# VisionDepth/VisionDepth3D

Measured on NVIDIA H100. Metric: end-to-end frames/sec (depth+stereo), higher is better.
Workload: dtype f16 GEMM operands, fp32 accumulate; DIBR fp32

## Files before the change

visiondepth3d_b200/csrc/depth_kernels.cu:

```cuda
#include <stdlib.h>

#include "depth_launch.h"
#include "umma_gemm.cuh"
#include "umma_attention.cuh"

namespace vd3d {

__global__ void __launch_bounds__(256) k_layernorm(const float* __restrict__ x, int rows, int D,
                                                   const float* __restrict__ gamma, const float* __restrict__ beta,
                                                   __half* __restrict__ out, int row_off, float eps) {
  int row = blockIdx.x * 8 + (threadIdx.x >> 5);
  int lane = threadIdx.x & 31;
  if (row >= rows) return;
  const float4* xr = (const float4*)(x + (size_t)(row + row_off) * D);
  float4 v[8];
  const int n = D / 128;
  float s = 0.f;
#pragma unroll
  for (int i = 0; i < 8; ++i)
    if (i < n) {
      v[i] = xr[lane + 32 * i];
      s += (v[i].x + v[i].y) + (v[i].z + v[i].w);
    }
  for (int o = 16; o; o >>= 1) s += __shfl_xor_sync(0xffffffffu, s, o);
  const float mean = s / (float)D;
  float q = 0.f;
#pragma unroll
  for (int i = 0; i < 8; ++i)
    if (i < n) {
      float a = v[i].x - mean, b = v[i].y - mean, c = v[i].z - mean, d = v[i].w - mean;
      q += (a * a + b * b) + (c * c + d * d);
    }
  for (int o = 16; o; o >>= 1) q += __shfl_xor_sync(0xffffffffu, q, o);
  const float rstd = rsqrtf(q / (float)D + eps);
  uint2* orow = (uint2*)(out + (size_t)row * D);
#pragma unroll
  for (int i = 0; i < 8; ++i)
    if (i < n) {
      const int c4 = lane + 32 * i;
      float4 g4 = ((const float4*)gamma)[c4], b4 = ((const float4*)beta)[c4];
      __half2 h0 = __floats2half2_rn((v[i].x - mean) * rstd * g4.x + b4.x, (v[i].y - mean) * rstd * g4.y + b4.y);
      __half2 h1 = __floats2half2_rn((v[i].z - mean) * rstd * g4.z + b4.z, (v[i].w - mean) * rstd * g4.w + b4.w);
      uint2 u;
      u.x = *(uint32_t*)&h0;
      u.y = *(uint32_t*)&h1;
      orow[c4] = u;
    }
}

__global__ void __launch_bounds__(256) k_patch_im2col(const float* __restrict__ px, int IH, int IW, int ph, int pw,
                                                      __half* __restrict__ A, int kpad) {
  int idx = blockIdx.x * 256 + threadIdx.x;
  int total = ph * pw * 588;
  if (idx >= total) return;
  int k = idx % 588, t = idx / 588;
  int c = k / 196, rr = k % 196, dy = rr / 14, dx = rr % 14;
  int py = t / pw, pxx = t % pw;
  float v = px[((size_t)c * IH + (py * 14 + dy)) * IW + (pxx * 14 + dx)];
  A[(size_t)t * kpad + k] = __float2half_rn(v);
}

__global__ void k_set_cls(float* __restrict__ x, const float* __restrict__ cls, const float* __restrict__ pos, int D) {
  int i = blockIdx.x * 256 + threadIdx.x;
  if (i < D) x[i] = cls[i] + pos[i];
}

__global__ void __launch_bounds__(256) k_im2col_s2(const __half* __restrict__ in, int H, int W, int C, int ldc,
                                                   __half* __restrict__ out, int OH, int OW) {
  size_t idx = (size_t)blockIdx.x * 256 + threadIdx.x;
  size_t total = (size_t)OH * OW * 9 * C;
  if (idx >= total) return;
  int c = idx % C;
  size_t r = idx / C;
  int tap = r % 9;
  size_t o = r / 9;
  int ox = o % OW, oy = o / OW;
  int iy = oy * 2 - 1 + tap / 3, ix = ox * 2 - 1 + tap % 3;
  __half v = __float2half_rn(0.f);
  if (iy >= 0 && iy < H && ix >= 0 && ix < W) v = in[((size_t)iy * W + ix) * ldc + c];
  out[idx] = v;
}

__global__ void __launch_bounds__(256) k_upsample_ac(const __half* __restrict__ in, int H, int W, int C,
                                                     __half* __restrict__ out, int OH, int OW) {
  size_t idx = (size_t)blockIdx.x * 256 + threadIdx.x;
  int c8 = C / 8;
  size_t total = (size_t)OH * OW * c8;
  if (idx >= total) return;
  int cg = idx % c8;
  size_t o = idx / c8;
  int ox = o % OW, oy = o / OW;
  float sy = (OH > 1) ? (float)(H - 1) / (float)(OH - 1) : 0.f;
  float sx = (OW > 1) ? (float)(W - 1) / (float)(OW - 1) : 0.f;
  float fy = sy * oy, fx = sx * ox;
  int y0 = (int)fy, x0 = (int)fx;
  int y1 = min(y0 + 1, H - 1), x1 = min(x0 + 1, W - 1);
  float ly = fy - y0, lx = fx - x0;
  const uint4* p00 = (const uint4*)(in + ((size_t)y0 * W + x0) * C) + cg;
  const uint4* p01 = (const uint4*)(in + ((size_t)y0 * W + x1) * C) + cg;
  const uint4* p10 = (const uint4*)(in + ((size_t)y1 * W + x0) * C) + cg;
  const uint4* p11 = (const uint4*)(in + ((size_t)y1 * W + x1) * C) + cg;
  uint4 a = *p00, b = *p01, c = *p10, d = *p11, r;
  const __half2* ha = (const __half2*)&a;
  const __half2* hb = (const __half2*)&b;
  const __half2* hc = (const __half2*)&c;
  const __half2* hd = (const __half2*)&d;
  __half2* hr = (__half2*)&r;
#pragma unroll
  for (int j = 0; j < 4; ++j) {
    float2 fa = __half22float2(ha[j]), fb = __half22float2(hb[j]), fc = __half22float2(hc[j]),
           fd = __half22float2(hd[j]);
    float t0x = fa.x + lx * (fb.x - fa.x), t0y = fa.y + lx * (fb.y - fa.y);
    float t1x = fc.x + lx * (fd.x - fc.x), t1y = fc.y + lx * (fd.y - fc.y);
    hr[j] = __floats2half2_rn(t0x + ly * (t1x - t0x), t0y + ly * (t1y - t0y));
  }
  ((uint4*)(out + o * C))[cg] = r;
}

__global__ void __launch_bounds__(256) k_relu_f16(const __half* __restrict__ in, __half* __restrict__ out, size_t n8) {
  size_t i = (size_t)blockIdx.x * 256 + threadIdx.x;
  if (i >= n8) return;
  uint4 a = ((const uint4*)in)[i];
  __half2* h = (__half2*)&a;
  const __half2 z = __floats2half2_rn(0.f, 0.f);
#pragma unroll
  for (int j = 0; j < 4; ++j) h[j] = __hmax2(h[j], z);
  ((uint4*)out)[i] = a;
}

__device__ __forceinline__ float cubic_aa(float x) {
  const float a = -0.5f;
  x = fabsf(x);
  if (x < 1.0f) return ((a + 2.0f) * x - (a + 3.0f)) * x * x + 1.0f;
  if (x < 2.0f) return (((x - 5.0f) * x + 8.0f) * x - 4.0f) * a;
  return 0.0f;
}

__global__ void __launch_bounds__(256) k_resize_aa_u8(const uint8_t* __restrict__ src, int IH, int IW,
                                                      uint8_t* __restrict__ dst, int OH, int OW, int axis_y,
                                                      int bgr_to_rgb) {
  int ox = blockIdx.x * 32 + (threadIdx.x & 31);
  int oy = blockIdx.y * 8 + (threadIdx.x >> 5);
  if (ox >= OW || oy >= OH) return;
  const int in_sz = axis_y ? IH : IW, out_sz = axis_y ? OH : OW, o = axis_y ? oy : ox;
  float scale = (float)in_sz / (float)out_sz;
  float support = (scale >= 1.0f) ? 2.0f * scale : 2.0f;
  float invscale = (scale >= 1.0f) ? 1.0f / scale : 1.0f;
  float center = scale * ((float)o + 0.5f);
  int xmin = max(0, (int)(center - support + 0.5f));
  int xmax = min(in_sz, (int)(center + support + 0.5f));
  float wsum = 0.f, acc[3] = {0.f, 0.f, 0.f};
  for (int j = xmin; j < xmax; ++j) {
    float w = cubic_aa(((float)j - center + 0.5f) * invscale);
    wsum += w;
    const uint8_t* q = axis_y ? src + ((size_t)j * IW + ox) * 3 : src + ((size_t)oy * IW + j) * 3;
    acc[0] += w * (float)q[0];
    acc[1] += w * (float)q[1];
    acc[2] += w * (float)q[2];
  }
  uint8_t* d = dst + ((size_t)oy * OW + ox) * 3;
#pragma unroll
  for (int c = 0; c < 3; ++c) {
    float v = acc[c] / wsum;
    int iv = __float2int_rn(v);
    iv = iv < 0 ? 0 : (iv > 255 ? 255 : iv);
    d[bgr_to_rgb ? 2 - c : c] = (uint8_t)iv;
  }
}

__global__ void __launch_bounds__(256) k_normalize_px(const uint8_t* __restrict__ rgb, int H, int W,
                                                      float* __restrict__ px) {
  int i = blockIdx.x * 256 + threadIdx.x;
  if (i >= H * W) return;
  const float mean[3] = {0.485f, 0.456f, 0.406f}, stdv[3] = {0.229f, 0.224f, 0.225f};
#pragma unroll
  for (int c = 0; c < 3; ++c) {
    float v = (float)rgb[(size_t)i * 3 + c] * (1.0f / 255.0f);
    px[(size_t)c * H * W + i] = (v - mean[c]) / stdv[c];
  }
}

__device__ __forceinline__ void cubic_coeffs(float t, float* c) {
  const float A = -0.75f;
  float x;
  x = t + 1.0f;
  c[0] = ((A * x - 5.0f * A) * x + 8.0f * A) * x - 4.0f * A;
  x = t;
  c[1] = ((A + 2.0f) * x - (A + 3.0f)) * x * x + 1.0f;
  x = 1.0f - t;
  c[2] = ((A + 2.0f) * x - (A + 3.0f)) * x * x + 1.0f;
  x = 2.0f - t;
  c[3] = ((A * x - 5.0f * A) * x + 8.0f * A) * x - 4.0f * A;
}
__device__ __forceinline__ unsigned f2ord(float f) {
  unsigned u = __float_as_uint(f);
  return (u & 0x80000000u) ? ~u : (u | 0x80000000u);
}
__device__ __forceinline__ float ord2f(unsigned u) {
  return __uint_as_float((u & 0x80000000u) ? (u & 0x7FFFFFFFu) : ~u);
}
__global__ void __launch_bounds__(256) k_depth_upsample_minmax(const float* __restrict__ d, int IH, int IW,
                                                               float* __restrict__ out, int OH, int OW,
                                                               unsigned* __restrict__ mm) {
  int ox = blockIdx.x * 32 + (threadIdx.x & 31);
  int oy = blockIdx.y * 8 + (threadIdx.x >> 5);
  float v = 0.f;
  bool ok = ox < OW && oy < OH;
  if (ok) {
    if (IH == OH && IW == OW) {
      v = d[(size_t)oy * IW + ox];
    } else {
      float sy = (float)IH / (float)OH, sx = (float)IW / (float)OW;
      float fy = sy * ((float)oy + 0.5f) - 0.5f, fx = sx * ((float)ox + 0.5f) - 0.5f;
      int iy = (int)floorf(fy), ix = (int)floorf(fx);
      float cy[4], cx[4];
      cubic_coeffs(fy - (float)iy, cy);
      cubic_coeffs(fx - (float)ix, cx);
      v = 0.f;
#pragma unroll
      for (int j = 0; j < 4; ++j) {
        int yy = min(max(iy - 1 + j, 0), IH - 1);
        float r = 0.f;
#pragma unroll
        for (int i = 0; i < 4; ++i) {
          int xx = min(max(ix - 1 + i, 0), IW - 1);
          r += cx[i] * d[(size_t)yy * IW + xx];
        }
        v += cy[j] * r;
      }
    }
    out[(size_t)oy * OW + ox] = v;
  }
  __shared__ float slo[8], shi[8];
  float lo = ok ? v : INFINITY, hi = ok ? v : -INFINITY;
  for (int o = 16; o; o >>= 1) {
    lo = fminf(lo, __shfl_xor_sync(0xffffffffu, lo, o));
    hi = fmaxf(hi, __shfl_xor_sync(0xffffffffu, hi, o));
  }
  if ((threadIdx.x & 31) == 0) {
    slo[threadIdx.x >> 5] = lo;
    shi[threadIdx.x >> 5] = hi;
  }
  __syncthreads();
  if (threadIdx.x == 0) {
    for (int i = 1; i < 8; ++i) {
      lo = fminf(lo, slo[i]);
      hi = fmaxf(hi, shi[i]);
    }
    if (lo <= hi) {
      atomicMin(&mm[0], f2ord(lo));
      atomicMax(&mm[1], f2ord(hi));
    }
  }
}
__global__ void k_minmax_reset(unsigned* mm) {
  mm[0] = 0xFFFFFFFFu;
  mm[1] = 0u;
}
__global__ void __launch_bounds__(256) k_depth_to_u8(const float* __restrict__ d, int n, const unsigned* __restrict__ mm,
                                                     uint8_t* __restrict__ out, int invert) {
  int i = blockIdx.x * 256 + threadIdx.x;
  if (i >= n) return;
  float lo = ord2f(mm[0]), hi = ord2f(mm[1]);
  float v = ((d[i] - lo) / (hi - lo + 1e-6f)) * 255.0f;
  int iv = (int)v;
  iv = iv < 0 ? 0 : (iv > 255 ? 255 : iv);
  out[i] = (uint8_t)(invert ? 255 - iv : iv);
}

__global__ void __launch_bounds__(256) k_add_relu_f16(const __half* __restrict__ a, const __half* __restrict__ b,
                                                      __half* __restrict__ sum, __half* __restrict__ sum_relu,
                                                      size_t n8) {
  size_t i = (size_t)blockIdx.x * 256 + threadIdx.x;
  if (i >= n8) return;
  uint4 ua = ((const uint4*)a)[i], ub = ((const uint4*)b)[i], us, ur;
  const __half2* ha = (const __half2*)&ua;
  const __half2* hb = (const __half2*)&ub;
  __half2* hs = (__half2*)&us;
  __half2* hr = (__half2*)&ur;
#pragma unroll
  for (int j = 0; j < 4; ++j) {
    float2 fa = __half22float2(ha[j]), fb = __half22float2(hb[j]);
    float sx = fa.x + fb.x, sy = fa.y + fb.y;
    hs[j] = __floats2half2_rn(sx, sy);
    hr[j] = __floats2half2_rn(fmaxf(sx, 0.f), fmaxf(sy, 0.f));
  }
  ((uint4*)sum)[i] = us;
  ((uint4*)sum_relu)[i] = ur;
}

void launch_preprocess(const uint8_t* frame_bgr, int H, int W, uint8_t* tmp_u8, uint8_t* rgb_u8, float* px, int OH,
                       int OW, cudaStream_t s) {
  dim3 g1((OW + 31) / 32, (H + 7) / 8), g2((OW + 31) / 32, (OH + 7) / 8);
  k_resize_aa_u8<<<g1, 256, 0, s>>>(frame_bgr, H, W, tmp_u8, H, OW, 0, 0);
  k_resize_aa_u8<<<g2, 256, 0, s>>>(tmp_u8, H, OW, rgb_u8, OH, OW, 1, 1);
  k_normalize_px<<<(OH * OW + 255) / 256, 256, 0, s>>>(rgb_u8, OH, OW, px);
}
void launch_depth_post(const float* depth, int IH, int IW, float* up, int OH, int OW, unsigned* mm, uint8_t* out_u8,
                       int invert, cudaStream_t s) {
  k_minmax_reset<<<1, 1, 0, s>>>(mm);
  dim3 g((OW + 31) / 32, (OH + 7) / 8);
  k_depth_upsample_minmax<<<g, 256, 0, s>>>(depth, IH, IW, up, OH, OW, mm);
  if (out_u8) k_depth_to_u8<<<(OH * OW + 255) / 256, 256, 0, s>>>(up, OH * OW, mm, out_u8, invert);
}
void launch_add_relu_f16(const __half* a, const __half* b, __half* sum, __half* sum_relu, size_t n, cudaStream_t s) {
  size_t n8 = n / 8;
  k_add_relu_f16<<<(unsigned)((n8 + 255) / 256), 256, 0, s>>>(a, b, sum, sum_relu, n8);
}
void launch_layernorm(const float* x, int rows, int D, const float* g, const float* b, __half* out, int row_off,
                      cudaStream_t s) {
  k_layernorm<<<(rows + 7) / 8, 256, 0, s>>>(x, rows, D, g, b, out, row_off, 1e-6f);
}
void launch_patch_im2col(const float* px, int IH, int IW, int ph, int pw, __half* A, int kpad, cudaStream_t s) {
  int total = ph * pw * 588;
  k_patch_im2col<<<(total + 255) / 256, 256, 0, s>>>(px, IH, IW, ph, pw, A, kpad);
}
void launch_set_cls(float* x, const float* cls, const float* pos, int D, cudaStream_t s) {
  k_set_cls<<<(D + 255) / 256, 256, 0, s>>>(x, cls, pos, D);
}
void launch_im2col_s2(const __half* in, int H, int W, int C, int ldc, __half* out, int OH, int OW, cudaStream_t s) {
  size_t total = (size_t)OH * OW * 9 * C;
  k_im2col_s2<<<(unsigned)((total + 255) / 256), 256, 0, s>>>(in, H, W, C, ldc, out, OH, OW);
}
void launch_upsample_ac(const __half* in, int H, int W, int C, __half* out, int OH, int OW, cudaStream_t s) {
  size_t total = (size_t)OH * OW * (C / 8);
  k_upsample_ac<<<(unsigned)((total + 255) / 256), 256, 0, s>>>(in, H, W, C, out, OH, OW);
}
__global__ void __launch_bounds__(256) k_sr_in(const uint8_t* __restrict__ bgr, __half* __restrict__ x, int npix) {
  int i = blockIdx.x * 256 + threadIdx.x;
  if (i >= npix) return;
  const uint8_t* q = bgr + (size_t)i * 3;
  uint4 z = make_uint4(0, 0, 0, 0);
  uint4* dst = (uint4*)(x + (size_t)i * 64);
  __align__(16) __half h4[8];
  h4[0] = __float2half_rn((float)q[2] / 255.0f);
  h4[1] = __float2half_rn((float)q[1] / 255.0f);
  h4[2] = __float2half_rn((float)q[0] / 255.0f);
#pragma unroll
  for (int k = 3; k < 8; ++k) h4[k] = __float2half_rn(0.f);
  dst[0] = *(uint4*)h4;
#pragma unroll
  for (int k = 1; k < 8; ++k) dst[k] = z;
}
__global__ void __launch_bounds__(256) k_sr_out(const float* __restrict__ conv, int ldc, const uint8_t* __restrict__ bgr,
                                                uint8_t* __restrict__ out, int h, int w) {
  int X = blockIdx.x * 32 + (threadIdx.x & 31);
  int Y = blockIdx.y * 8 + (threadIdx.x >> 5);
  if (X >= 4 * w || Y >= 4 * h) return;
  const int y = Y >> 2, x = X >> 2, sub = (Y & 3) * 4 + (X & 3);
  const float* cv = conv + ((size_t)y * w + x) * ldc + sub;
  const uint8_t* q = bgr + ((size_t)y * w + x) * 3;
  uint8_t* o = out + ((size_t)Y * 4 * w + X) * 3;
#pragma unroll
  for (int c = 0; c < 3; ++c) {
    float v = cv[c * 16] + ((float)q[2 - c] / 255.0f);
    v = fminf(fmaxf(v, 0.f), 1.f) * 255.0f;
    o[2 - c] = (uint8_t)(int)v;
  }
}
void launch_sr_in(const uint8_t* bgr, __half* x, int npix, cudaStream_t s) {
  k_sr_in<<<(npix + 255) / 256, 256, 0, s>>>(bgr, x, npix);
}
void launch_sr_out(const float* conv, int ldc, const uint8_t* bgr, uint8_t* out, int h, int w, cudaStream_t s) {
  dim3 g((4 * w + 31) / 32, (4 * h + 7) / 8);
  k_sr_out<<<g, 256, 0, s>>>(conv, ldc, bgr, out, h, w);
}

void launch_relu_f16(const __half* in, __half* out, size_t n, cudaStream_t s) {
  size_t n8 = n / 8;
  k_relu_f16<<<(unsigned)((n8 + 255) / 256), 256, 0, s>>>(in, out, n8);
}

template <int BN, int STAGES>
static cudaError_t launch_gemm_t(const CUtensorMap& a, const CUtensorMap& b, const GemmArgs& g, dim3 grid,
                                 cudaStream_t s) {
  static bool attr_set = false;
  constexpr int smem = GemmSmem<BN, STAGES>::kTotal;
  if (!attr_set) {
    cudaError_t e = cudaFuncSetAttribute(k_umma_gemm<BN, STAGES>, cudaFuncAttributeMaxDynamicSharedMemorySize, smem);
    if (e != cudaSuccess) return e;
    attr_set = true;
  }
  k_umma_gemm<BN, STAGES><<<grid, kGemmThreads, smem, s>>>(a, b, g);
  return cudaGetLastError();
}

cudaError_t launch_attention(const CUtensorMap& q, const CUtensorMap& k, const CUtensorMap& v, int ntok, int dmodel,
                             __half* out, int heads, int images, int npad, cudaStream_t s) {
  static bool attr_set = false;
  if (!attr_set) {
    cudaError_t e = cudaFuncSetAttribute(k_umma_attention, cudaFuncAttributeMaxDynamicSharedMemorySize, kAttnSmem);
    if (e != cudaSuccess) return e;
    attr_set = true;
  }
  AttnArgs a;
  a.ntok = ntok;
  a.dmodel = dmodel;
  a.out = out;
  a.heads = heads;
  a.npad = npad;
  dim3 grid((ntok + 127) / 128, heads * images);
  k_umma_attention<<<grid, kAttnThreads, kAttnSmem, s>>>(q, k, v, a);
  return cudaGetLastError();
}

static int sm_count() {
  static int sms = 0;
  if (!sms) {
    int dev = 0;
    cudaGetDevice(&dev);
    if (cudaDeviceGetAttribute(&sms, cudaDevAttrMultiProcessorCount, dev) != cudaSuccess || sms <= 0) sms = 132;
  }
  return sms;
}

cudaError_t launch_gemm_variant(int variant, const CUtensorMap& a, const CUtensorMap& b, const GemmArgs& g_in,
                                int m_tiles, int batch, cudaStream_t s) {
  GemmArgs g = g_in;
  g.nt = (g.N + 127) / 128;
  g.mt = m_tiles;
  g.nz = batch;
  const int total = g.nt * g.mt * g.nz, sms = sm_count();
  dim3 grid(total < sms ? total : sms, 1, 1);
  switch (variant) {
    case 0: return launch_gemm_t<128, 4>(a, b, g, grid, s);
    case 1: return launch_gemm_t<128, 3>(a, b, g, grid, s);
    case 2: return launch_gemm_t<128, 2>(a, b, g, grid, s);
    default: return cudaErrorInvalidValue;
  }
}

cudaError_t launch_gemm(int bn, const CUtensorMap& a, const CUtensorMap& b, const GemmArgs& g_in, int m_tiles,
                        int batch, cudaStream_t s) {
  GemmArgs g = g_in;
  g.nt = (g.N + bn - 1) / bn;
  g.mt = m_tiles;
  g.nz = batch;
  const int total = g.nt * g.mt * g.nz, sms = sm_count();
  dim3 grid(total < sms ? total : sms, 1, 1);
  switch (bn) {
    case 128: return launch_gemm_t<128, 4>(a, b, g, grid, s);
    case 64: return launch_gemm_t<64, 6>(a, b, g, grid, s);
    case 32: return launch_gemm_t<32, 6>(a, b, g, grid, s);
    default: return cudaErrorInvalidValue;
  }
}

}
```

visiondepth3d_b200/csrc/umma_attention.cuh:

```cuda
#pragma once
#include "umma_gemm.cuh"

namespace vd3d {

struct AttnArgs {
  int ntok;
  int dmodel;
  __half* out;
  int heads;
  int npad;
};

constexpr int kAttnThreads = 384;
constexpr int kAttnKS = 2;
constexpr int kAttnSmem = 16384  + kAttnKS * (16384  + 16384 ) + 1024  + 256 ;

namespace umma {
__device__ __forceinline__ float quad_max(float x) {
  x = fmaxf(x, __shfl_xor_sync(0xffffffffu, x, 1));
  return fmaxf(x, __shfl_xor_sync(0xffffffffu, x, 2));
}
__device__ __forceinline__ float quad_sum(float x) {
  x += __shfl_xor_sync(0xffffffffu, x, 1);
  return x + __shfl_xor_sync(0xffffffffu, x, 2);
}
__device__ __forceinline__ uint32_t pack_h2(float a, float b) {
  __half2 h = __floats2half2_rn(a, b);
  return *(uint32_t*)&h;
}
}

__global__ void __launch_bounds__(kAttnThreads, 1)
k_umma_attention(const __grid_constant__ CUtensorMap tmQ, const __grid_constant__ CUtensorMap tmK,
                 const __grid_constant__ CUtensorMap tmV, const AttnArgs g) {
  extern __shared__ uint8_t smem_raw[];
  const uint32_t sm = (umma::smem_u32(smem_raw) + 1023u) & ~1023u;
  const uint32_t sQ = sm, sK = sm + 16384, sV = sK + kAttnKS * 16384;
  const uint32_t bars = sV + kAttnKS * 16384;
  const uint32_t q_full = bars, kv_full = bars + 8, kv_empty = kv_full + 8 * kAttnKS;

  const int warp = threadIdx.x >> 5, lane = threadIdx.x & 31;
  const int qblk = blockIdx.x, zq = blockIdx.y, h = zq % g.heads, img = zq / g.heads;
  const int T = (g.ntok + 127) / 128;

  if (warp == 0 && lane == 0) {
    umma::prefetch_tmap(&tmQ);
    umma::prefetch_tmap(&tmK);
    umma::prefetch_tmap(&tmV);
    umma::mbar_init(q_full, 1);
    for (int i = 0; i < kAttnKS; ++i) {
      umma::mbar_init(kv_full + 8 * i, 1);
      umma::mbar_init(kv_empty + 8 * i, 2);
    }
    umma::fence_barrier_init();
  }
  __syncthreads();

  if (warp < 4) {
    if (warp == 0 && lane == 0) {
      umma::mbar_expect_tx(q_full, 16384);
      umma::tma_load_3d(sQ, &tmQ, q_full, 0, qblk * 128, zq);
      for (int t = 0; t < T; ++t) {
        const int ks = t % kAttnKS;
        umma::mbar_wait(kv_empty + 8 * ks, ((t / kAttnKS) & 1) ^ 1);
        const uint32_t fb = kv_full + 8 * ks;
        umma::mbar_expect_tx(fb, 32768);
        umma::tma_load_3d(sK + ks * 16384, &tmK, fb, 0, t * 128, zq);
        const uint32_t dst = sV + ks * 16384;
        umma::tma_load_3d(dst, &tmV, fb, t * 128, 0, zq);
        umma::tma_load_3d(dst + 8192, &tmV, fb, t * 128 + 64, 0, zq);
      }
    }
    return;
  }

  const int wg = (warp >> 2) - 1;
  const int wq = warp & 3;
  const float L2E = 1.4426950408889634f;
  const int cq = 2 * (lane & 3);
  float o[32];
#pragma unroll
  for (int i = 0; i < 32; ++i) o[i] = 0.f;
  float m_run[2] = {-INFINITY, -INFINITY}, l_run[2] = {0.f, 0.f};

  umma::mbar_wait(q_full, 0);
  const uint64_t dq = umma::make_desc(sQ + (uint32_t)(wg * 64 * 128));
  for (int t = 0; t < T; ++t) {
    const int ks = t % kAttnKS;
    umma::mbar_wait(kv_full + 8 * ks, (t / kAttnKS) & 1);
    float s[64];
    {
      const uint64_t dk = umma::make_desc(sK + ks * 16384);
      umma::wgmma_fence();
#pragma unroll
      for (int k = 0; k < 4; ++k) umma::wgmma_m64n128_ss(s, dq + (uint64_t)(2 * k), dk + (uint64_t)(2 * k), k ? 1u : 0u);
      umma::wgmma_commit();
      umma::wgmma_wait<0>();
      umma::fence_regs(s);
    }
    const int nvalid = g.ntok - t * 128;
    float mx[2] = {-INFINITY, -INFINITY};
#pragma unroll
    for (int j = 0; j < 16; ++j)
#pragma unroll
      for (int i = 0; i < 4; ++i) {
        if (nvalid < 128 && 8 * j + cq + (i & 1) >= nvalid) s[4 * j + i] = -INFINITY;
        mx[i >> 1] = fmaxf(mx[i >> 1], s[4 * j + i]);
      }
    float scale[2], mref[2];
#pragma unroll
    for (int rr = 0; rr < 2; ++rr) {
      const float m_new = fmaxf(m_run[rr], umma::quad_max(mx[rr]) * L2E);
      scale[rr] = umma::ex2_fast(m_run[rr] - m_new);
      m_run[rr] = m_new;
      mref[rr] = m_new - 8.0f;
    }
    float ls[2] = {0.f, 0.f};
    uint32_t p[32];
#pragma unroll
    for (int j = 0; j < 16; ++j) {
      const float p0 = umma::ex2_fast(fmaf(s[4 * j + 0], L2E, -mref[0]));
      const float p1 = umma::ex2_fast(fmaf(s[4 * j + 1], L2E, -mref[0]));
      const float p2 = umma::ex2_fast(fmaf(s[4 * j + 2], L2E, -mref[1]));
      const float p3 = umma::ex2_fast(fmaf(s[4 * j + 3], L2E, -mref[1]));
      p[2 * j] = umma::pack_h2(p0, p1);
      p[2 * j + 1] = umma::pack_h2(p2, p3);
      const float2 h0 = __half22float2(*(const __half2*)&p[2 * j]), h1 = __half22float2(*(const __half2*)&p[2 * j + 1]);
      ls[0] += h0.x + h0.y;
      ls[1] += h1.x + h1.y;
    }
#pragma unroll
    for (int rr = 0; rr < 2; ++rr) l_run[rr] = l_run[rr] * scale[rr] + ls[rr];
#pragma unroll
    for (int j = 0; j < 8; ++j) {
      o[4 * j + 0] *= scale[0];
      o[4 * j + 1] *= scale[0];
      o[4 * j + 2] *= scale[1];
      o[4 * j + 3] *= scale[1];
    }
    umma::fence_regs(o);
    umma::wgmma_fence();
#pragma unroll
    for (int kk = 0; kk < 8; ++kk) {
      const uint32_t a[4] = {p[4 * kk], p[4 * kk + 1], p[4 * kk + 2], p[4 * kk + 3]};
      const uint64_t db = umma::make_desc(sV + ks * 16384 + (kk >> 2) * 8192) + (uint64_t)(2 * (kk & 3));
      umma::wgmma_m64n64_rs(o, a, db, 1u);
    }
    umma::wgmma_commit();
    umma::wgmma_wait<0>();
    umma::fence_regs(o);
    if ((threadIdx.x & 127) == 0) umma::mbar_arrive(kv_empty + 8 * ks);
  }

  float inv[2];
#pragma unroll
  for (int rr = 0; rr < 2; ++rr) inv[rr] = 1.0f / umma::quad_sum(l_run[rr]);
  const int r0 = qblk * 128 + wg * 64 + wq * 16 + (lane >> 2);
#pragma unroll
  for (int rr = 0; rr < 2; ++rr) {
    const int m = r0 + 8 * rr;
    if (m >= g.ntok) continue;
    __half* dst = g.out + ((size_t)img * g.npad + m) * g.dmodel + h * 64 + cq;
#pragma unroll
    for (int j = 0; j < 8; ++j)
      *(uint32_t*)(dst + 8 * j) = umma::pack_h2(o[4 * j + 2 * rr] * inv[rr], o[4 * j + 2 * rr + 1] * inv[rr]);
  }
}

}
```

Baseline: 318.6.

## Make attention persistent with QK/PV software pipelining and register rebalancing

```diff
diff --git a/visiondepth3d_b200/csrc/depth_kernels.cu b/visiondepth3d_b200/csrc/depth_kernels.cu
--- a/visiondepth3d_b200/csrc/depth_kernels.cu
+++ b/visiondepth3d_b200/csrc/depth_kernels.cu
@@ -385,6 +385,16 @@
   return cudaGetLastError();
 }
 
+static int sm_count() {
+  static int sms = 0;
+  if (!sms) {
+    int dev = 0;
+    cudaGetDevice(&dev);
+    if (cudaDeviceGetAttribute(&sms, cudaDevAttrMultiProcessorCount, dev) != cudaSuccess || sms <= 0) sms = 132;
+  }
+  return sms;
+}
+
 cudaError_t launch_attention(const CUtensorMap& q, const CUtensorMap& k, const CUtensorMap& v, int ntok, int dmodel,
                              __half* out, int heads, int images, int npad, cudaStream_t s) {
   static bool attr_set = false;
@@ -399,19 +409,9 @@
   a.out = out;
   a.heads = heads;
   a.npad = npad;
-  dim3 grid((ntok + 127) / 128, heads * images);
-  k_umma_attention<<<grid, kAttnThreads, kAttnSmem, s>>>(q, k, v, a);
+  a.items = (ntok + 127) / 128 * heads * images;
+  k_umma_attention<<<std::min(a.items, sm_count()), kAttnThreads, kAttnSmem, s>>>(q, k, v, a);
   return cudaGetLastError();
-}
-
-static int sm_count() {
-  static int sms = 0;
-  if (!sms) {
-    int dev = 0;
-    cudaGetDevice(&dev);
-    if (cudaDeviceGetAttribute(&sms, cudaDevAttrMultiProcessorCount, dev) != cudaSuccess || sms <= 0) sms = 132;
-  }
-  return sms;
 }
 
 cudaError_t launch_gemm_variant(int variant, const CUtensorMap& a, const CUtensorMap& b, const GemmArgs& g_in,
diff --git a/visiondepth3d_b200/csrc/umma_attention.cuh b/visiondepth3d_b200/csrc/umma_attention.cuh
--- a/visiondepth3d_b200/csrc/umma_attention.cuh
+++ b/visiondepth3d_b200/csrc/umma_attention.cuh
@@ -9,11 +9,16 @@
   __half* out;
   int heads;
   int npad;
+  int items;
 };
 
 constexpr int kAttnThreads = 384;
-constexpr int kAttnKS = 2;
-constexpr int kAttnSmem = 16384  + kAttnKS * (16384  + 16384 ) + 1024  + 256 ;
+constexpr int kAttnKS = 3;
+constexpr int kAttnSmem = 2 * 16384  + kAttnKS * (16384  + 16384 ) + 1024  +
+                          256 ;
+constexpr int kAttnProducerRegs = 24;
+constexpr int kAttnConsumerRegs = 240;
+static_assert(128 * kAttnProducerRegs + 256 * kAttnConsumerRegs <= 384 * 168, "register file overcommitted");
 
 namespace umma {
 __device__ __forceinline__ float quad_max(float x) {
@@ -27,6 +32,73 @@
 __device__ __forceinline__ uint32_t pack_h2(float a, float b) {
   __half2 h = __floats2half2_rn(a, b);
   return *(uint32_t*)&h;
+}
+
+__device__ __forceinline__ void attn_qk(float (&s)[64], uint64_t dq, uint32_t sk) {
+  const uint64_t dk = make_desc(sk);
+#pragma unroll
+  for (int k = 0; k < 4; ++k) wgmma_m64n128_ss(s, dq + (uint64_t)(2 * k), dk + (uint64_t)(2 * k), k ? 1u : 0u);
+}
+__device__ __forceinline__ void attn_pv(float (&o)[32], const uint32_t (&p)[32], uint32_t sv) {
+#pragma unroll
+  for (int kk = 0; kk < 8; ++kk) {
+    const uint32_t a[4] = {p[4 * kk], p[4 * kk + 1], p[4 * kk + 2], p[4 * kk + 3]};
+    const uint64_t db = make_desc(sv + (kk >> 2) * 8192) + (uint64_t)(2 * (kk & 3));
+    wgmma_m64n64_rs(o, a, db, 1u);
+  }
+}
+template <bool kMask>
+__device__ __forceinline__ void attn_softmax(float (&s)[64], int nvalid, int cq, float (&m_run)[2], float (&l_run)[2],
+                                             float (&scale)[2]) {
+  const float L2E = 1.4426950408889634f;
+  float mx[2] = {-INFINITY, -INFINITY};
+#pragma unroll
+  for (int j = 0; j < 16; ++j)
+#pragma unroll
+    for (int i = 0; i < 4; ++i) {
+      if (kMask && 8 * j + cq + (i & 1) >= nvalid) s[4 * j + i] = -INFINITY;
+      mx[i >> 1] = fmaxf(mx[i >> 1], s[4 * j + i]);
+    }
+  float mref[2];
+#pragma unroll
+  for (int rr = 0; rr < 2; ++rr) {
+    const float m_new = fmaxf(m_run[rr], quad_max(mx[rr]) * L2E);
+    scale[rr] = ex2_fast(m_run[rr] - m_new);
+    m_run[rr] = m_new;
+    mref[rr] = m_new - 8.0f;
+  }
+  float ls[2] = {0.f, 0.f};
+#pragma unroll
+  for (int j = 0; j < 16; ++j) {
+    const float p0 = ex2_fast(fmaf(s[4 * j + 0], L2E, -mref[0]));
+    const float p1 = ex2_fast(fmaf(s[4 * j + 1], L2E, -mref[0]));
+    const float p2 = ex2_fast(fmaf(s[4 * j + 2], L2E, -mref[1]));
+    const float p3 = ex2_fast(fmaf(s[4 * j + 3], L2E, -mref[1]));
+    const uint32_t u0 = pack_h2(p0, p1), u1 = pack_h2(p2, p3);
+    const float2 h0 = __half22float2(*(const __half2*)&u0), h1 = __half22float2(*(const __half2*)&u1);
+    s[4 * j + 0] = h0.x;
+    s[4 * j + 1] = h0.y;
+    s[4 * j + 2] = h1.x;
+    s[4 * j + 3] = h1.y;
+    ls[0] += h0.x + h0.y;
+    ls[1] += h1.x + h1.y;
+  }
+#pragma unroll
+  for (int rr = 0; rr < 2; ++rr) l_run[rr] = l_run[rr] * scale[rr] + ls[rr];
+}
+__device__ __forceinline__ void attn_pack(const float (&s)[64], uint32_t (&p)[32]) {
+#pragma unroll
+  for (int j = 0; j < 16; ++j) {
+    p[2 * j] = pack_h2(s[4 * j + 0], s[4 * j + 1]);
+    p[2 * j + 1] = pack_h2(s[4 * j + 2], s[4 * j + 3]);
+  }
+}
+__device__ __forceinline__ void attn_softmax_tile(float (&s)[64], int nvalid, int cq, float (&m_run)[2],
+                                                  float (&l_run)[2], float (&scale)[2]) {
+  if (nvalid < 128)
+    attn_softmax<true>(s, nvalid, cq, m_run, l_run, scale);
+  else
+    attn_softmax<false>(s, nvalid, cq, m_run, l_run, scale);
 }
 }
 
@@ -35,19 +107,22 @@
                  const __grid_constant__ CUtensorMap tmV, const AttnArgs g) {
   extern __shared__ uint8_t smem_raw[];
   const uint32_t sm = (umma::smem_u32(smem_raw) + 1023u) & ~1023u;
-  const uint32_t sQ = sm, sK = sm + 16384, sV = sK + kAttnKS * 16384;
+  const uint32_t sQ = sm, sK = sm + 2 * 16384, sV = sK + kAttnKS * 16384;
   const uint32_t bars = sV + kAttnKS * 16384;
-  const uint32_t q_full = bars, kv_full = bars + 8, kv_empty = kv_full + 8 * kAttnKS;
+  const uint32_t q_full = bars, q_empty = bars + 16, kv_full = bars + 32, kv_empty = kv_full + 8 * kAttnKS;
 
   const int warp = threadIdx.x >> 5, lane = threadIdx.x & 31;
-  const int qblk = blockIdx.x, zq = blockIdx.y, h = zq % g.heads, img = zq / g.heads;
-  const int T = (g.ntok + 127) / 128;
+  const int QB = (g.ntok + 127) / 128;
+  const int T = QB;
 
   if (warp == 0 && lane == 0) {
     umma::prefetch_tmap(&tmQ);
     umma::prefetch_tmap(&tmK);
     umma::prefetch_tmap(&tmV);
-    umma::mbar_init(q_full, 1);
+    for (int i = 0; i < 2; ++i) {
+      umma::mbar_init(q_full + 8 * i, 1);
+      umma::mbar_init(q_empty + 8 * i, 2);
+    }
     for (int i = 0; i < kAttnKS; ++i) {
       umma::mbar_init(kv_full + 8 * i, 1);
       umma::mbar_init(kv_empty + 8 * i, 2);
@@ -57,114 +132,108 @@
   __syncthreads();
 
   if (warp < 4) {
+    asm volatile("setmaxnreg.dec.sync.aligned.u32 %0;" ::"n"(kAttnProducerRegs));
     if (warp == 0 && lane == 0) {
-      umma::mbar_expect_tx(q_full, 16384);
-      umma::tma_load_3d(sQ, &tmQ, q_full, 0, qblk * 128, zq);
-      for (int t = 0; t < T; ++t) {
-        const int ks = t % kAttnKS;
-        umma::mbar_wait(kv_empty + 8 * ks, ((t / kAttnKS) & 1) ^ 1);
-        const uint32_t fb = kv_full + 8 * ks;
-        umma::mbar_expect_tx(fb, 32768);
-        umma::tma_load_3d(sK + ks * 16384, &tmK, fb, 0, t * 128, zq);
-        const uint32_t dst = sV + ks * 16384;
-        umma::tma_load_3d(dst, &tmV, fb, t * 128, 0, zq);
-        umma::tma_load_3d(dst + 8192, &tmV, fb, t * 128 + 64, 0, zq);
+      int kit = 0;
+      int li = 0;
+      for (int item = blockIdx.x; item < g.items; item += gridDim.x, ++li) {
+        const int qblk = item % QB, zq = item / QB, qb = li & 1;
+        umma::mbar_wait(q_empty + 8 * qb, ((li >> 1) & 1) ^ 1);
+        umma::mbar_expect_tx(q_full + 8 * qb, 16384);
+        umma::tma_load_3d(sQ + qb * 16384, &tmQ, q_full + 8 * qb, 0, qblk * 128, zq);
+        for (int t = 0; t < T; ++t, ++kit) {
+          const int ks = kit % kAttnKS;
+          umma::mbar_wait(kv_empty + 8 * ks, ((kit / kAttnKS) & 1) ^ 1);
+          const uint32_t fb = kv_full + 8 * ks;
+          umma::mbar_expect_tx(fb, 32768);
+          umma::tma_load_3d(sK + ks * 16384, &tmK, fb, 0, t * 128, zq);
+          const uint32_t dst = sV + ks * 16384;
+          umma::tma_load_3d(dst, &tmV, fb, t * 128, 0, zq);
+          umma::tma_load_3d(dst + 8192, &tmV, fb, t * 128 + 64, 0, zq);
+        }
       }
     }
     return;
   }
 
+  asm volatile("setmaxnreg.inc.sync.aligned.u32 %0;" ::"n"(kAttnConsumerRegs));
   const int wg = (warp >> 2) - 1;
   const int wq = warp & 3;
-  const float L2E = 1.4426950408889634f;
+  const bool lead = (threadIdx.x & 127) == 0;
   const int cq = 2 * (lane & 3);
-  float o[32];
-#pragma unroll
-  for (int i = 0; i < 32; ++i) o[i] = 0.f;
-  float m_run[2] = {-INFINITY, -INFINITY}, l_run[2] = {0.f, 0.f};
-
-  umma::mbar_wait(q_full, 0);
-  const uint64_t dq = umma::make_desc(sQ + (uint32_t)(wg * 64 * 128));
-  for (int t = 0; t < T; ++t) {
-    const int ks = t % kAttnKS;
-    umma::mbar_wait(kv_full + 8 * ks, (t / kAttnKS) & 1);
+  int kit = 0, li = 0;
+  for (int item = blockIdx.x; item < g.items; item += gridDim.x, ++li) {
+    const int qblk = item % QB, zq = item / QB, h = zq % g.heads, img = zq / g.heads, qb = li & 1;
+    float o[32];
+#pragma unroll
+    for (int i = 0; i < 32; ++i) o[i] = 0.f;
+    float m_run[2] = {-INFINITY, -INFINITY}, l_run[2] = {0.f, 0.f}, scale[2];
     float s[64];
+    uint32_t p[32];
+
+    umma::mbar_wait(q_full + 8 * qb, (li >> 1) & 1);
+    const uint64_t dq = umma::make_desc(sQ + qb * 16384 + (uint32_t)(wg * 64 * 128));
+    umma::mbar_wait(kv_full + 8 * (kit % kAttnKS), (kit / kAttnKS) & 1);
+    umma::wgmma_fence();
+    umma::attn_qk(s, dq, sK + (kit % kAttnKS) * 16384);
+    umma::wgmma_commit();
+    umma::wgmma_wait<0>();
+    umma::fence_regs(s);
+    umma::attn_softmax_tile(s, g.ntok, cq, m_run, l_run, scale);
+    umma::attn_pack(s, p);
+    for (int t = 1; t < T; ++t) {
+      const int kprev = (kit + t - 1) % kAttnKS, kcur = (kit + t) % kAttnKS;
+      umma::mbar_wait(kv_full + 8 * kcur, ((kit + t) / kAttnKS) & 1);
+      umma::fence_regs(o);
+      umma::wgmma_fence();
+      umma::attn_qk(s, dq, sK + kcur * 16384);
+      umma::wgmma_commit();
+      umma::attn_pv(o, p, sV + kprev * 16384);
+      umma::wgmma_commit();
+      umma::wgmma_wait<1>();
+      umma::fence_regs(s);
+      umma::attn_softmax_tile(s, g.ntok - t * 128, cq, m_run, l_run, scale);
+      umma::wgmma_wait<0>();
+      umma::fence_regs(o);
+      if (lead) umma::mbar_arrive(kv_empty + 8 * kprev);
+#pragma unroll
+      for (int j = 0; j < 8; ++j) {
+        o[4 * j + 0] *= scale[0];
+        o[4 * j + 1] *= scale[0];
+        o[4 * j + 2] *= scale[1];
+        o[4 * j + 3] *= scale[1];
+      }
+      umma::attn_pack(s, p);
+    }
     {
-      const uint64_t dk = umma::make_desc(sK + ks * 16384);
+      const int klast = (kit + T - 1) % kAttnKS;
+      umma::fence_regs(o);
       umma::wgmma_fence();
-#pragma unroll
-      for (int k = 0; k < 4; ++k) umma::wgmma_m64n128_ss(s, dq + (uint64_t)(2 * k), dk + (uint64_t)(2 * k), k ? 1u : 0u);
+      umma::attn_pv(o, p, sV + klast * 16384);
       umma::wgmma_commit();
       umma::wgmma_wait<0>();
-      umma::fence_regs(s);
-    }
-    const int nvalid = g.ntok - t * 128;
-    float mx[2] = {-INFINITY, -INFINITY};
-#pragma unroll
-    for (int j = 0; j < 16; ++j)
-#pragma unroll
-      for (int i = 0; i < 4; ++i) {
-        if (nvalid < 128 && 8 * j + cq + (i & 1) >= nvalid) s[4 * j + i] = -INFINITY;
-        mx[i >> 1] = fmaxf(mx[i >> 1], s[4 * j + i]);
+      umma::fence_regs(o);
+      if (lead) {
+        umma::mbar_arrive(kv_empty + 8 * klast);
+        umma::mbar_arrive(q_empty + 8 * qb);
       }
-    float scale[2], mref[2];
+    }
+    kit += T;
+
+    float inv[2];
+#pragma unroll
+    for (int rr = 0; rr < 2; ++rr) inv[rr] = 1.0f / umma::quad_sum(l_run[rr]);
+    const int r0 = qblk * 128 + wg * 64 + wq * 16 + (lane >> 2);
 #pragma unroll
     for (int rr = 0; rr < 2; ++rr) {
-      const float m_new = fmaxf(m_run[rr], umma::quad_max(mx[rr]) * L2E);
-      scale[rr] = umma::ex2_fast(m_run[rr] - m_new);
-      m_run[rr] = m_new;
-      mref[rr] = m_new - 8.0f;
-    }
-    float ls[2] = {0.f, 0.f};
-    uint32_t p[32];
-#pragma unroll
-    for (int j = 0; j < 16; ++j) {
-      const float p0 = umma::ex2_fast(fmaf(s[4 * j + 0], L2E, -mref[0]));
-      const float p1 = umma::ex2_fast(fmaf(s[4 * j + 1], L2E, -mref[0]));
-      const float p2 = umma::ex2_fast(fmaf(s[4 * j + 2], L2E, -mref[1]));
-      const float p3 = umma::ex2_fast(fmaf(s[4 * j + 3], L2E, -mref[1]));
-      p[2 * j] = umma::pack_h2(p0, p1);
-      p[2 * j + 1] = umma::pack_h2(p2, p3);
-      const float2 h0 = __half22float2(*(const __half2*)&p[2 * j]), h1 = __half22float2(*(const __half2*)&p[2 * j + 1]);
-      ls[0] += h0.x + h0.y;
-      ls[1] += h1.x + h1.y;
-    }
-#pragma unroll
-    for (int rr = 0; rr < 2; ++rr) l_run[rr] = l_run[rr] * scale[rr] + ls[rr];
-#pragma unroll
-    for (int j = 0; j < 8; ++j) {
-      o[4 * j + 0] *= scale[0];
-      o[4 * j + 1] *= scale[0];
-      o[4 * j + 2] *= scale[1];
-      o[4 * j + 3] *= scale[1];
-    }
-    umma::fence_regs(o);
-    umma::wgmma_fence();
-#pragma unroll
-    for (int kk = 0; kk < 8; ++kk) {
-      const uint32_t a[4] = {p[4 * kk], p[4 * kk + 1], p[4 * kk + 2], p[4 * kk + 3]};
-      const uint64_t db = umma::make_desc(sV + ks * 16384 + (kk >> 2) * 8192) + (uint64_t)(2 * (kk & 3));
-      umma::wgmma_m64n64_rs(o, a, db, 1u);
-    }
-    umma::wgmma_commit();
-    umma::wgmma_wait<0>();
-    umma::fence_regs(o);
-    if ((threadIdx.x & 127) == 0) umma::mbar_arrive(kv_empty + 8 * ks);
-  }
-
-  float inv[2];
-#pragma unroll
-  for (int rr = 0; rr < 2; ++rr) inv[rr] = 1.0f / umma::quad_sum(l_run[rr]);
-  const int r0 = qblk * 128 + wg * 64 + wq * 16 + (lane >> 2);
-#pragma unroll
-  for (int rr = 0; rr < 2; ++rr) {
-    const int m = r0 + 8 * rr;
-    if (m >= g.ntok) continue;
-    __half* dst = g.out + ((size_t)img * g.npad + m) * g.dmodel + h * 64 + cq;
-#pragma unroll
-    for (int j = 0; j < 8; ++j)
-      *(uint32_t*)(dst + 8 * j) = umma::pack_h2(o[4 * j + 2 * rr] * inv[rr], o[4 * j + 2 * rr + 1] * inv[rr]);
-  }
-}
-
-}
+      const int m = r0 + 8 * rr;
+      if (m >= g.ntok) continue;
+      __half* dst = g.out + ((size_t)img * g.npad + m) * g.dmodel + h * 64 + cq;
+#pragma unroll
+      for (int j = 0; j < 8; ++j)
+        *(uint32_t*)(dst + 8 * j) = umma::pack_h2(o[4 * j + 2 * rr] * inv[rr], o[4 * j + 2 * rr + 1] * inv[rr]);
+    }
+  }
+}
+
+}
```

Result: faster. 330.5 (median of 6 runs) (+3.8%).
